# WoojuLee24/OA-DG

Hardware: AMD Instinct MI355X
Metric: images/sec training, Faster R-CNN R50-FPN + OA-DG, 1024x2048 (higher is better)
Workload: dtype bf16

## Files before the change

include/oadg_hip.h:

```cpp
#ifndef OADG_HIP_H
#define OADG_HIP_H

#include <stddef.h>
#include <stdint.h>

#ifdef __cplusplus
extern "C" {
#endif

size_t oadg_supcon_workspace_bytes(int B, int D);
int oadg_supcon_fwd(const float* feats, const int64_t* labels, int B, int D, int n_labels, int ori_size,
                    int rp_size, float temper, int min_samples, float loss_weight, void* workspace,
                    size_t workspace_bytes, float* out_loss, void* stream);
int oadg_supcon_bwd(const int64_t* labels, int B, int D, int n_labels, int ori_size, int rp_size,
                    float temper, float loss_weight, const float* grad_out, void* workspace,
                    size_t workspace_bytes, float* dfeats, void* stream);
int oadg_supcon_status(const void* workspace_host_copy);

size_t oadg_cls_loss_workspace_bytes(void);
int oadg_ce_jsd_fwd(const float* logits, const int64_t* labels, const float* weights, long R, int C,
                    int mode, float avg_factor, float loss_weight, float lambda_jsd, void* workspace,
                    size_t workspace_bytes, float* out3, void* stream);
int oadg_ce_jsd_bwd(const float* logits, const int64_t* labels, const float* weights, long R, int C,
                    int mode, float avg_factor, float loss_weight, float lambda_jsd, const float* grad_out,
// ... 146 lines not shown

int oadg_png_size(const char* path, int* height, int* width);
int oadg_png_decode_bgr(const char* path, uint8_t* out, int H, int W);

int oadg_glass_shuffle_u8(uint8_t* img, int H, int W, int C, int delta, int iters, const int32_t* dxdy);
int oadg_chamfer_l2_5x5(const uint8_t* src, int H, int W, float* dist);

int oadg_resize_bilinear_u8(const uint8_t* src, int H, int W, int C, uint8_t* dst, int Hn, int Wn, void* stream);
int oadg_flip_u8(const uint8_t* src, int H, int W, int C, uint8_t* dst, int direction, void* stream);

int oadg_conv2d_nhwc_bf16(const void* x, const void* w, const float* bias, const void* residual, void* y,
                          const void* zeros16, int N, int H, int W, int C, int K, int R, int S, int stride,
                          int pad, int dil, int relu, void* stream);

int oadg_conv2d_nhwc_bf16_variant(const void* x, const void* w, const float* bias, const void* residual, void* y,
                                  const void* zeros16, int N, int H, int W, int C, int K, int R, int S, int stride,
                                  int pad, int dil, int relu, int variant, void* stream);
int oadg_conv2d_nhwc_bf16_ex(const void* x, const void* w, const float* bias, const void* residual, void* y,
                             const void* zeros16, int N, int H, int W, int C, int K, int R, int S, int stride, int pad,
                             int dil, int relu, int variant, const void* mask, float* colsum_part,
                             const void* mask_bits, void* relu_bits_out, void* stream);
long oadg_conv2d_pixel_tiles(int N, int H, int W, int C, int K, int R, int S, int stride, int pad, int dil,
                             int variant);
int oadg_colsum_reduce(const float* part, long rows, int K, float* out, void* stream);
typedef struct oadg_colsum_job {
    const float* part;
    float* out;
    float* dgamma;
    const float* mean;
    const float* var;
    int rows, K, first_block;
    float eps;
} oadg_colsum_job;
int oadg_colsum_reduce_multi(const oadg_colsum_job* jobs_dev, int n, int total_blocks, void* stream);
int oadg_conv2d_auto_variant(int N, int H, int W, int C, int K, int R, int S, int stride, int pad, int dil);
size_t oadg_conv2d_wgrad_workspace_bytes(int N, int Ho, int Wo, int C, int K, int R, int S);
int oadg_conv2d_wgrad_variant(int N, int Ho, int Wo, int C, int K, int R, int S);
int oadg_conv2d_wgrad_nhwc_bf16(const void* x, const void* dy, float* dw, const void* zeros16, void* workspace,
                                size_t workspace_bytes, int N, int H, int W, int C, int K, int R, int S,
                                int stride, int pad, int dil, void* stream);

int oadg_conv2d_wgrad_parts_nhwc_bf16(const void* x, const void* dy, const void* zeros16, void* workspace,
                                      size_t workspace_bytes, int N, int H, int W, int C, int K, int R, int S,
                                      int stride, int pad, int dil, int* splits, void* stream);
int oadg_prep_conv_weights_bwd_parts(const float* part, int splits, const float* gbias, const float* w,
                                     const float* scale, const float* mean, const float* var, float eps, int K, int C,
// ... 191 lines not shown
```

oa-dg_amd/_lib.py:

```python
import ctypes
import os
from ctypes import (POINTER, Structure, c_char_p, c_double, c_float, c_int, c_int64, c_long, c_size_t, c_void_p)

_HERE = os.path.dirname(os.path.abspath(__file__))
LIB_PATH = os.environ.get('OADG_HIP_LIB') or os.path.join(_HERE, 'csrc', 'liboadg_hip.so')
_lib = None

vp, ci, cf, cl, cs, cd = c_void_p, c_int, c_float, c_long, c_size_t, c_double


class RpnLevel(Structure):
    _fields_ = [('deltas', c_void_p), ('sN', c_long), ('sC', c_long), ('sH', c_long), ('sW', c_long), ('anchors', c_void_p),
                ('scores', c_void_p), ('index', c_void_p), ('H', c_int), ('W', c_int), ('A', c_int), ('k', c_int),
                ('dtype', c_int), ('first', c_int)]


class RpnLossLevel(Structure):
    _fields_ = [('y', c_void_p), ('gy', c_void_p), ('sN', c_long), ('sC', c_long), ('sH', c_long), ('sW', c_long),
                ('H', c_int), ('W', c_int), ('Cy', c_int), ('first', c_long), ('pix0', c_long)]


class RoiAssignImage(Structure):
    _fields_ = [('proposals', c_void_p), ('gt_bboxes', c_void_p), ('gt_labels', c_void_p), ('stride', c_int),
                ('num_gts', c_int)]
# ... 37 lines not shown
                                vp, ci, ci, ci, ci, ci, vp, vp, vp]),
    'oadg_roi_align_bwd': (ci, [POINTER(vp), POINTER(ci), POINTER(ci), POINTER(cf), ci, ci, ci, ci, cf,
                                vp, ci, ci, ci, ci, ci, vp, vp, vp]),
    'oadg_roi_order_keys': (ci, [vp, ci, ci, ci, cf, vp, vp]),
    'oadg_roi_order': (ci, [vp, ci, ci, ci, cf, vp, vp, vp]),
    'oadg_roi_align_bwd_tiles': (ci, [POINTER(vp), POINTER(ci), POINTER(ci), POINTER(cf), ci, ci, ci, cf, vp, ci, ci, ci,
                                      ci, ci, vp, vp, vp, vp, vp]),
    'oadg_rpn_loss_workspace_bytes': (cs, []),
    'oadg_rpn_loss_fwd': (ci, [vp, ci, ci, ci, cl, ci, vp, vp, vp, vp, cf, cf, cf, cf, vp, cs, vp, vp]),
    'oadg_rpn_loss_bwd': (ci, [vp, ci, ci, ci, cl, ci, vp, vp, vp, vp, cf, cf, cf, cf, vp, vp, vp]),
    'oadg_rpn_decode': (ci, [vp, ci, ci, vp, vp, cf, vp, ci, cf, vp, vp, vp, vp]),
    'oadg_rpn_order': (ci, [vp, ci, ci, vp, vp, vp, vp, vp, vp, vp, vp]),
    'oadg_rpn_gather': (ci, [ci, ci, ci, vp, vp, vp, vp, vp, vp, vp]),
    'oadg_rpn_topk_workspace_bytes': (cs, [POINTER(ci), ci, ci, ci]),
    'oadg_rpn_topk': (ci, [POINTER(vp), POINTER(cl), POINTER(ci), ci, ci, ci, ci, POINTER(vp), POINTER(vp), vp, cs, vp]),
    'oadg_nms_workspace_bytes': (cs, [ci, ci]),
    'oadg_nms_batched': (ci, [vp, vp, ci, ci, cf, ci, vp, cs, vp, vp, vp]),
    'oadg_resize_bilinear_u8': (ci, [vp, ci, ci, ci, vp, ci, ci, vp]),
    'oadg_flip_u8': (ci, [vp, ci, ci, ci, vp, ci, vp]),
    'oadg_conv2d_nhwc_bf16': (ci, [vp, vp, vp, vp, vp, vp] + [ci] * 11 + [vp]),
    'oadg_conv2d_auto_variant': (ci, [ci] * 10),
    'oadg_conv2d_nhwc_bf16_ex': (ci, [vp, vp, vp, vp, vp, vp] + [ci] * 12 + [vp, vp, vp, vp, vp]),
    'oadg_conv2d_pixel_tiles': (cl, [ci] * 11),
    'oadg_colsum_reduce': (ci, [vp, cl, ci, vp, vp]),
    'oadg_conv2d_nhwc_bf16_variant': (ci, [vp, vp, vp, vp, vp, vp] + [ci] * 12 + [vp]),
    'oadg_conv2d_wgrad_workspace_bytes': (cs, [ci] * 7),
    'oadg_conv2d_wgrad_variant': (ci, [ci] * 7),
    'oadg_conv2d_wgrad_nhwc_bf16': (ci, [vp, vp, vp, vp, vp, cs] + [ci] * 10 + [vp]),
    'oadg_conv2d_wgrad_parts_nhwc_bf16': (ci, [vp, vp, vp, vp, cs] + [ci] * 10 + [POINTER(ci), vp]),
    'oadg_prep_conv_weights_bwd_parts': (ci, [vp, ci, vp, vp, vp, vp, vp, cf, ci, ci, ci, ci, vp, vp, ci, vp]),
    'oadg_prep_conv_weights': (ci, [vp, vp, vp, vp, vp, cf, vp, ci, ci, ci, ci, vp, vp, vp, vp, ci, ci, vp]),
    'oadg_prep_conv_weights_multi': (ci, [vp, ci, ci, vp]),
    'oadg_prep_conv_weights_multi_blocks': (ci, [ci, ci, ci, ci]),
    'oadg_conv2d_nhwc_bf16_scatter': (ci, [vp, vp, vp, vp, vp, vp] + [ci] * 18 + [vp, vp, vp, vp]),
    'oadg_conv2d_dgrad_s2_nhwc_bf16': (ci, [vp, vp, vp, vp, vp, ci, ci, ci, ci, ci, ci, ci, ci, vp, vp, vp, vp]),
    'oadg_prep_conv_weights_bwd': (ci, [vp, vp, vp, vp, vp, vp, cf, ci, ci, ci, ci, vp, vp, ci, vp]),
    'oadg_relu_bias_bwd_workspace_bytes': (ctypes.c_size_t, [cl, ci]),
    'oadg_relu_bias_bwd': (ci, [vp, ci, vp, vp, vp, vp, ctypes.c_size_t, cl, ci, vp]),
    'oadg_stem_conv7x7s2_nhwc_bf16': (ci, [vp, vp, vp, ci, ci, ci, vp]),
    'oadg_bias_relu_maxpool_nhwc_bf16': (ci, [vp, vp, vp, ci, ci, ci, ci, vp]),
    'oadg_fpn_topdown_fwd': (ci, [vp, vp, vp, ci, ci, ci, ci, ci, ci, vp]),
    'oadg_fpn_topdown_bwd': (ci, [vp, vp, ci, ci, ci, ci, ci, ci, vp]),
    'oadg_max_iou_assign_workspace_bytes': (ctypes.c_size_t, [ci, ci]),
    'oadg_max_iou_assign': (ci, [vp, cl, vp, vp, vp, vp, ci, ci, ci, cf, cf, cf, cf, ci, vp, ctypes.c_size_t, vp, vp, vp,
                                 vp, vp]),
    'oadg_sample_select_workspace_bytes': (ctypes.c_size_t, [ci, cl]),
# ... 101 lines not shown
```

oa-dg_amd/backbones.py:

```python
import torch
import torch.nn as nn
import torch.nn.functional as F
from torch.nn.modules.batchnorm import _BatchNorm

import os

from . import hip_conv
from .layers import Conv2d, build_norm_layer, constant_init, conv_bn, kaiming_init
from .registry import BACKBONES


STEM_KERNEL = os.environ.get('OADG_STEM_KERNEL', '1') == '1'


class Bottleneck(nn.Module):
    expansion = 4

    def __init__(self, inplanes, planes, stride=1, dilation=1, downsample=None, style='pytorch',
                 norm_cfg=dict(type='BN')):
        super().__init__()
        assert style in ('pytorch', 'caffe')
        s1, s2 = (1, stride) if style == 'pytorch' else (stride, 1)
        self.conv1 = Conv2d(inplanes, planes, 1, stride=s1, bias=False)
        _, self.bn1 = build_norm_layer(norm_cfg, planes)
        self.conv2 = Conv2d(planes, planes, 3, stride=s2, padding=dilation, dilation=dilation, bias=False)
        _, self.bn2 = build_norm_layer(norm_cfg, planes)
        self.conv3 = Conv2d(planes, planes * self.expansion, 1, bias=False)
        _, self.bn3 = build_norm_layer(norm_cfg, planes * self.expansion)
        self.relu = nn.ReLU(inplace=True)
        self.downsample = downsample

    def forward(self, x):
        out = hip_conv.frozen_bottleneck(x, self)
        if out is not None:
            return out
        t_in = getattr(x, '_oadg_token', None)
        if hip_conv.tokens_ok(x, self.conv1, self.conv2, self.conv3) and not (self.bn1.training or self.bn2.training
                                                                              or self.bn3.training):
            t_a, t_b, t_out = hip_conv.GradToken(), hip_conv.GradToken(), hip_conv.GradToken()
            if not x.requires_grad or (self.downsample is not None and
                                       not hip_conv.tokens_ok(x, self.downsample[0])):
                t_in = None
            out = conv_bn(x, self.conv1, self.bn1, relu=True, in_token=t_in, out_token=t_a)
            out = conv_bn(out, self.conv2, self.bn2, relu=True, in_token=t_a, out_token=t_b)
            if self.downsample is not None:
                identity = conv_bn(x, self.downsample[0], self.downsample[1], dep_token=t_in)
                out = conv_bn(out, self.conv3, self.bn3, relu=True, residual=identity, in_token=t_b, out_token=t_out)
            else:
                out = conv_bn(out, self.conv3, self.bn3, relu=True, residual=x, in_token=t_b, out_token=t_out,
                              res_token=t_in)
            out._oadg_token = t_out
            return out
        identity = x
        if self.downsample is not None:
            identity = conv_bn(x, self.downsample[0], self.downsample[1])
        out = conv_bn(x, self.conv1, self.bn1, relu=True)
        out = conv_bn(out, self.conv2, self.bn2, relu=True)
        return conv_bn(out, self.conv3, self.bn3, relu=True, residual=identity)


def make_res_layer(inplanes, planes, num_blocks, stride, dilation, style, norm_cfg):
    downsample = None
    if stride != 1 or inplanes != planes * Bottleneck.expansion:
        downsample = nn.Sequential(
            Conv2d(inplanes, planes * Bottleneck.expansion, 1, stride=stride, bias=False),
            build_norm_layer(norm_cfg, planes * Bottleneck.expansion)[1])
    blocks = [Bottleneck(inplanes, planes, stride, dilation, downsample, style, norm_cfg)]
    inplanes = planes * Bottleneck.expansion
    for _ in range(1, num_blocks):
        blocks.append(Bottleneck(inplanes, planes, 1, dilation, None, style, norm_cfg))
    return nn.Sequential(*blocks)


@BACKBONES.register_module()
class ResNet(nn.Module):
    arch_settings = {50: (3, 4, 6, 3), 101: (3, 4, 23, 3), 152: (3, 8, 36, 3)}

    def __init__(self, depth, in_channels=3, stem_channels=None, base_channels=64, num_stages=4,
                 strides=(1, 2, 2, 2), dilations=(1, 1, 1, 1), out_indices=(0, 1, 2, 3), style='pytorch',
                 deep_stem=False, avg_down=False, frozen_stages=-1, conv_cfg=None,
                 norm_cfg=dict(type='BN', requires_grad=True), norm_eval=True, dcn=None,
                 stage_with_dcn=(False, False, False, False), plugins=None, with_cp=False,
                 zero_init_residual=True, pretrained=None, init_cfg=None):
        super().__init__()
        if depth not in self.arch_settings:
            raise KeyError(f'invalid depth {depth} for resnet (bottleneck depths only)')
        assert not deep_stem and not avg_down and dcn is None and plugins is None and not with_cp
        assert 1 <= num_stages <= 4 and len(strides) == len(dilations) == num_stages
        assert max(out_indices) < num_stages
        self.depth, self.out_indices, self.frozen_stages = depth, out_indices, frozen_stages
        self.norm_eval, self.zero_init_residual, self.init_cfg = norm_eval, zero_init_residual, init_cfg
        stem_channels = stem_channels or base_channels
        self.conv1 = Conv2d(in_channels, stem_channels, 7, stride=2, padding=3, bias=False)
        _, self.bn1 = build_norm_layer(norm_cfg, stem_channels)
# ... 101 lines not shown
```

oa-dg_amd/csrc/conv_mfma.hip:

```cpp
#include <algorithm>
#include <vector>
#include "common.h"
#include <type_traits>
#include <stdlib.h>
#include "oadg_hip.h"

namespace {

constexpr int BM = 128, BN = 128, BK = 64;

struct ConvArgs {
    const unsigned short* x;
    const unsigned short* w;
    const float* bias;
    const unsigned short* res;
    unsigned short* y;
    const unsigned short* zeros;
    const unsigned short* mask;
    const unsigned char* bits_in;
    unsigned char* bits_out;
    float* colsum;
    int N, H, W, C, K, R, S, Ho, Wo, stride, pad, dil, relu;
    long M;
    int scatter, OH, OW, osh, osw, oph, opw;
// ... 512 lines not shown
int launch_pw_stream(const ConvArgs& a, hipStream_t st) {
    using Geo = PwGeo<C>;
    const int ncol = a.K / (4 * Geo::KPW);
    const bool res = a.res != nullptr, bin = a.bits_in != nullptr, bout = a.bits_out != nullptr;
#define OADG_PWS(RE, BI, BO)                                                                                       \
    do {                                                                                                           \
        static bool attr = false;                                                                                  \
        if (!attr) {                                                                                               \
            hipError_t e = hipFuncSetAttribute((const void*)conv_pw_stream_kernel<C, RE, BI, BO>,                  \
                                               hipFuncAttributeMaxDynamicSharedMemorySize, Geo::LDS);              \
            if (e != hipSuccess) return (int)e;                                                                    \
            attr = true;                                                                                           \
        }                                                                                                          \
        hipLaunchKernelGGL((conv_pw_stream_kernel<C, RE, BI, BO>), dim3(Geo::GRID), dim3(256), Geo::LDS, st, a, ncol); \
    } while (0)
    if (res && bin && !bout) OADG_PWS(true, true, false);
    else if (res && !bin && bout) OADG_PWS(true, false, true);
    else if (res && !bin && !bout) OADG_PWS(true, false, false);
    else if (!res && bin && !bout) OADG_PWS(false, true, false);
    else if (!res && !bin && bout) OADG_PWS(false, false, true);
    else if (!res && !bin && !bout) OADG_PWS(false, false, false);
    else return OADG_EARG;
#undef OADG_PWS
    return OADG_OK;
}

constexpr int TM = 256, TN = 256;
constexpr int HALF_BYTES = 128 * BK * 2;
constexpr int BUF_BYTES = 4 * HALF_BYTES;

typedef float f32x4v __attribute__((ext_vector_type(4)));

struct TapState {
    int t, r, s, rs, c0;
};

template <bool POST, int NW>
__global__ __launch_bounds__(512) void conv_igemm256_kernel(ConvArgs a) {
    constexpr int TNW = NW * 128;
    extern __shared__ __attribute__((aligned(16))) unsigned char smem[];
    const int tid = threadIdx.x, lane = tid & 63;
    const int wave = __builtin_amdgcn_readfirstlane(tid >> 6);
    const int wr = wave >> 2, wc = wave & 3;
    const int n_tiles = a.K / TNW;
    const long m_tiles = (a.M + TM - 1) / TM;
    const long bid = blockIdx.x;
// ... 363 lines not shown
}
}

extern "C" int oadg_conv2d_nhwc_bf16(const void* x, const void* w, const float* bias, const void* residual,
                                     void* y, const void* zeros16, int N, int H, int W, int C, int K, int R,
                                     int S, int stride, int pad, int dil, int relu, void* stream) {
    return conv_launch(x, w, bias, residual, y, zeros16, N, H, W, C, K, R, S, stride, pad, dil, relu, 0, stream);
}

extern "C" int oadg_conv2d_auto_variant(int N, int H, int W, int C, int K, int R, int S, int stride, int pad, int dil) {
    if (N < 1 || H < 1 || W < 1 || R < 1 || S < 1 || stride < 1 || dil < 1 || pad < 0) return 0;
    if (C % BK != 0 || K % 64 != 0) return 0;
    const int Ho = (H + 2 * pad - dil * (R - 1) - 1) / stride + 1, Wo = (W + 2 * pad - dil * (S - 1) - 1) / stride + 1;
    if (Ho < 1 || Wo < 1) return 0;
    return auto_variant((long)N * Ho * Wo, H, W, C, K, R * S * (C / BK), R, S, stride, pad);
}

extern "C" int oadg_conv2d_nhwc_bf16_ex(const void* x, const void* w, const float* bias, const void* residual,
                                        void* y, const void* zeros16, int N, int H, int W, int C, int K, int R, int S,
                                        int stride, int pad, int dil, int relu, int variant, const void* mask,
                                        float* colsum_part, const void* mask_bits, void* relu_bits_out, void* stream) {
    return conv_launch(x, w, bias, residual, y, zeros16, N, H, W, C, K, R, S, stride, pad, dil, relu, variant, stream,
                       mask, colsum_part, nullptr, mask_bits, relu_bits_out);
}

extern "C" int oadg_conv2d_nhwc_bf16_scatter(const void* x, const void* w, const float* bias, const void* residual,
                                             void* y, const void* zeros16, int N, int H, int W, int C, int K, int R,
                                             int S, int pad, int dil, int relu, int out_h, int out_w, int OH, int OW,
                                             int osh, int osw, int oph, int opw, const void* mask,
                                             float* colsum_part, const void* mask_bits, void* stream) {
    const int sc[8] = {out_h, out_w, OH, OW, osh, osw, oph, opw};
    return conv_launch(x, w, bias, residual, y, zeros16, N, H, W, C, K, R, S, 1, pad, dil, relu, 3, stream, mask,
                       colsum_part, sc, mask_bits, nullptr);
}

extern "C" int oadg_conv2d_dgrad_s2_nhwc_bf16(const void* dy, const void* wt, const void* residual, void* dx,
                                              const void* zeros16, int N, int Ho, int Wo, int K, int C, int R, int H, int W,
                                              const void* mask, float* colsum_part, const void* mask_bits, void* stream) {
    if (!dy || !wt || !dx || !zeros16 || N < 1 || Ho < 1 || Wo < 1 || H < 1 || W < 1 || (R != 3 && R != 1)) return OADG_EARG;
    if (K % BK != 0 || C % 64 != 0 || (mask_bits && C % 8 != 0)) return OADG_EARG;
    static const int cls_tab[4][5] = {{0, 0, 1, 1, 0}, {0, 1, 1, 2, 1}, {1, 0, 2, 1, 3}, {1, 1, 2, 2, 5}};
    S2Args g;
    ConvArgs& a = g.base;
    a.x = (const unsigned short*)dy; a.w = nullptr; a.bias = nullptr; a.res = (const unsigned short*)residual;
    a.y = (unsigned short*)dx; a.zeros = (const unsigned short*)zeros16; a.mask = (const unsigned short*)mask;
    a.bits_in = (const unsigned char*)mask_bits; a.bits_out = nullptr; a.colsum = nullptr;
// ... 1218 lines not shown
```

oa-dg_amd/hip_conv.py:

```python
import ctypes
import os

import numpy as np
import torch

from . import _lib
from ._lib import check, ptr, stream_ptr

_ZEROS = {}
USE_HIP_WGRAD = 'auto'
TIMERS = None
TIMERS_ONLY_VARIANT = None


def _timed(family):
    if TIMERS is None:
        return False
    only = TIMERS_ONLY_VARIANT
    return only is None or family == only or (isinstance(only, (set, frozenset, tuple, list)) and family in only)


def _wgrad_events(x16, gy16, K, R, S):
    if TIMERS is None:
        return None
# ... 831 lines not shown
        cache_on._prepared = (key, out)
    return out


class GradToken:
    __slots__ = ('extra', 'colsum', 'grad_ptr', 'bits', 'armed', 'closed', 'masked')

    def __init__(self, masked=True):
        self.extra = self.colsum = self.grad_ptr = self.bits = None
        self.armed = self.closed = False
        self.masked = masked


RELU_BITS = True
DEPOSIT = True


def y_numel(x, w, stride, pad, dil):
    N, _, H, W = x.shape
    K, _, R, S = w.shape
    return N * K * ((H + 2 * pad - dil * (R - 1) - 1) // stride + 1) * ((W + 2 * pad - dil * (S - 1) - 1) // stride + 1)


class _Conv2dMFMA(torch.autograd.Function):

    @staticmethod
    def forward(ctx, x, wf, bias, residual, wt, stride, pad, dil, relu, in_token, out_token, res_token, dep_token=None,
                res_up=False):
        x16 = _nhwc_bf16(x)
        if in_token is not None and wt is not None and stride == 1:
            in_token.armed = True
        r16 = _nhwc_bf16(residual) if residual is not None else None
        bits = None
        if relu and out_token is not None and RELU_BITS and wf.shape[0] % 8 == 0:
            bits = out_token.bits = torch.empty((y_numel(x16, wf, stride, pad, dil) // 8,), dtype=torch.uint8,
                                                device=x16.device)
        y = conv_forward(x16, wf, bias, r16, stride, pad, dil, relu, bits_out=bits, res_up=bool(res_up))
        ctx.res_up = tuple(r16.shape) if res_up else None
        ctx.save_for_backward(x16, wf, wt, y if relu else None)
        ctx.cfg = (stride, pad, dil, bias is not None, x.dtype, residual.dtype if residual is not None else None)
        ctx.tokens = (in_token, out_token, res_token, dep_token)
        ctx.wtoken = getattr(wf, '_oadg_wtoken', None)
        if ctx.wtoken is not None:
            ctx.wtoken.uses += 1
            ent = ctx.wtoken.entry
            if ent is not None and DEFER_WGRAD and SHARED_GROUP:
                K_, C_, R_, S_ = wf.shape
                work = wgrad_work(y.shape[0], y.shape[2], y.shape[3], C_, K_, R_, S_)
                if ent.expect_step != _STEP:
                    ent.expect_step, ent.expect_jobs, ent.shared = _STEP, 0, []
                if ctx.wtoken.deferrable and 0 < work < WGRAD_SMALL and C_ * R_ * S_ <= 36000 and x16.numel() < 2 ** 32 and \
                        _hip_wgrad(K_, C_, R_, y.shape[0] * y.shape[2] * y.shape[3]):
                    ent.expect_jobs += 1
        return y

    @staticmethod
    def backward(ctx, gy):
        x16, wf, wt, y = ctx.saved_tensors
        stride, pad, dil, has_bias, xdt, rdt = ctx.cfg
        in_token, out_token, res_token, dep_token = ctx.tokens
        K, C, R, S = wf.shape
        want_b = has_bias and ctx.needs_input_grad[2]
        gb = None
        if out_token is not None and out_token.grad_ptr is not None and out_token.grad_ptr == gy.data_ptr() and \
                gy.dtype == torch.bfloat16 and gy.is_contiguous(memory_format=torch.channels_last):
            gb = out_token.colsum if want_b else None
            want_b = False
            if pending_colsum(gb) is not None and not (ctx.wtoken is not None and ctx.wtoken.uses == 1):
                resolve_colsum(gb)
        elif (y is not None or want_b) and gy.dtype in (torch.bfloat16, torch.float32) and K % 8 == 0 and \
                gy.is_contiguous(memory_format=torch.channels_last):
            gy, gb = relu_bias_bwd(gy, y, want_b)
            want_b = False
        else:
            gy = _nhwc_bf16(gy)
            if y is not None:
# ... 29 lines not shown
            need_x = False
        if need_x and wt is not None and stride == 2:
            if in_token is not None and extra is None and in_token.masked:
                mb = in_token.bits
                gx, in_token.colsum = conv_dgrad_s2(gy, wt, x16.shape, R, mask=None if mb is not None else x16,
                                                    want_colsum=True, mask_bits=mb)
                in_token.grad_ptr = gx.data_ptr()
            else:
                gx = conv_dgrad_s2(gy, wt, x16.shape, R)
            need_x = False
        elif need_x and wt is not None:
            if in_token is not None:
                mb = in_token.bits if in_token.masked else None
                gx, in_token.colsum = conv_forward(gy, wt, None, extra, 1, dil * (R - 1) - pad, dil, False,
                                                   mask=x16 if (mb is None and in_token.masked) else None,
                                                   want_colsum=True, mask_bits=mb)
                in_token.grad_ptr = gx.data_ptr()
                extra = None
            else:
                gx = conv_forward(gy, wt, None, None, 1, dil * (R - 1) - pad, dil, False)
            need_x = False
        gw = None
        if need_w and x16.numel() < 2 ** 32 and _hip_wgrad(K, C, R, gy.shape[0] * gy.shape[2] * gy.shape[3]):
            wtok = ctx.wtoken
            work = wgrad_work(gy.shape[0], gy.shape[2], gy.shape[3], C, K, R, S) if DEFER_WGRAD else 0
            if wtok is not None and wtok.uses == 1 and wtok.deferrable and 0 < work < WGRAD_SMALL and C * R * S <= 36000:
                wtok.parts = _WgradJob(x16, gy, K, R, S, stride, pad, dil)
                gw = _dummy_grad(wf)
            elif wtok is not None and wtok.uses == 1 and C * R * S * 4 <= 12000:
                wtok.parts = conv_wgrad_parts(x16, gy, K, R, S, stride, pad, dil)
                gw = _dummy_grad(wf)
            else:
                gw = conv_wgrad(x16, gy, K, R, S, stride, pad, dil)
            need_w = False
            if want_b:
                gb = gy.float().sum((0, 2, 3))
                want_b = False
        if need_x or need_w or want_b:
            outs = torch.ops.aten.convolution_backward(
                gy, x16, wf, [K] if has_bias else None, [stride, stride], [pad, pad], [dil, dil], False, [0, 0],
                1, [need_x, need_w, want_b])
            if gx is None:
                gx = outs[0]
            if outs[1] is not None:
                gw = outs[1]
            if outs[2] is not None:
                gb = outs[2].float()
        if gx is not None and extra is not None:
            gx = gx + extra.to(gx.dtype)
        gres = None
        if rdt is not None and ctx.needs_input_grad[3]:
            if res_token is not None:
                res_token.extra = gy
            else:
                gres = gy.to(rdt)
            if ctx.res_up is not None:
                ts = ctx.res_up
                g16 = _nhwc_bf16(gy)
                gres = torch.empty(ts, dtype=torch.bfloat16, device=gy.device, memory_format=torch.channels_last)
                check(_lib.lib().oadg_fpn_topdown_bwd(ptr(g16), ptr(gres), g16.shape[0], g16.shape[2], g16.shape[3], ts[2],
                                                      ts[3], g16.shape[1], stream_ptr()), 'oadg_fpn_topdown_bwd')
                gres = gres.to(rdt)
        return (gx.to(xdt) if gx is not None else None), gw, gb, gres, None, None, None, None, None, None, None, None, None, None


NARROW_HEAD = os.environ.get('OADG_NARROW_HEAD', '1') == '1'


def narrow_params(w_cat, b_cat):
    KN, C = w_cat.shape[0], w_cat.shape[1]
    with torch.no_grad():
        w16 = torch.zeros((16, C), dtype=torch.bfloat16, device=w_cat.device)
        w16[:KN].copy_(w_cat.detach().reshape(KN, C))
        wt16 = w16.t().contiguous()
        b16 = torch.zeros((16,), dtype=torch.float32, device=w_cat.device)
        if b_cat is not None:
            b16[:KN].copy_(b_cat.detach())
    return w16, wt16, b16


def _n16_launch(kind, M, C, extra_bytes, fn):
    if TIMERS is None or not _timed('n16'):
        return fn()
    e0, e1 = torch.cuda.Event(enable_timing=True), torch.cuda.Event(enable_timing=True)
    e0.record()
    r = fn()
# ... 192 lines not shown
```

Measured before the change: 145.5.

## Fuse consecutive bottleneck 1x1 convs (conv3 + next conv1) into one streaming kernel

```diff
diff --git a/include/oadg_hip.h b/include/oadg_hip.h
--- a/include/oadg_hip.h
+++ b/include/oadg_hip.h
@@ -192,6 +192,11 @@
                              const void* mask_bits, void* relu_bits_out, void* stream);
 long oadg_conv2d_pixel_tiles(int N, int H, int W, int C, int K, int R, int S, int stride, int pad, int dil,
                              int variant);
+int oadg_conv_pw_pair_ok(long M, int C);
+int oadg_conv_pw_pair_nhwc_bf16(const void* x, const void* w1, const float* b1, const void* res, void* t,
+                                const void* t_bits_in, void* t_bits_out, float* t_colsum, const void* w2, const float* b2,
+                                void* y, const void* y_bits_in, void* y_bits_out, float* y_colsum, const void* zeros16,
+                                long M, int C, int bwd, void* stream);
 int oadg_colsum_reduce(const float* part, long rows, int K, float* out, void* stream);
 typedef struct oadg_colsum_job {
     const float* part;
diff --git a/oa-dg_amd/_lib.py b/oa-dg_amd/_lib.py
--- a/oa-dg_amd/_lib.py
+++ b/oa-dg_amd/_lib.py
@@ -83,6 +83,8 @@
     'oadg_conv2d_auto_variant': (ci, [ci] * 10),
     'oadg_conv2d_nhwc_bf16_ex': (ci, [vp, vp, vp, vp, vp, vp] + [ci] * 12 + [vp, vp, vp, vp, vp]),
     'oadg_conv2d_pixel_tiles': (cl, [ci] * 11),
+    'oadg_conv_pw_pair_ok': (ci, [cl, ci]),
+    'oadg_conv_pw_pair_nhwc_bf16': (ci, [vp] * 15 + [cl, ci, ci, vp]),
     'oadg_colsum_reduce': (ci, [vp, cl, ci, vp, vp]),
     'oadg_conv2d_nhwc_bf16_variant': (ci, [vp, vp, vp, vp, vp, vp] + [ci] * 12 + [vp]),
     'oadg_conv2d_wgrad_workspace_bytes': (cs, [ci] * 7),
diff --git a/oa-dg_amd/backbones.py b/oa-dg_amd/backbones.py
--- a/oa-dg_amd/backbones.py
+++ b/oa-dg_amd/backbones.py
@@ -34,29 +34,62 @@
         out = hip_conv.frozen_bottleneck(x, self)
         if out is not None:
             return out
-        t_in = getattr(x, '_oadg_token', None)
-        if hip_conv.tokens_ok(x, self.conv1, self.conv2, self.conv3) and not (self.bn1.training or self.bn2.training
-                                                                              or self.bn3.training):
-            t_a, t_b, t_out = hip_conv.GradToken(), hip_conv.GradToken(), hip_conv.GradToken()
-            if not x.requires_grad or (self.downsample is not None and
-                                       not hip_conv.tokens_ok(x, self.downsample[0])):
-                t_in = None
-            out = conv_bn(x, self.conv1, self.bn1, relu=True, in_token=t_in, out_token=t_a)
-            out = conv_bn(out, self.conv2, self.bn2, relu=True, in_token=t_a, out_token=t_b)
-            if self.downsample is not None:
-                identity = conv_bn(x, self.downsample[0], self.downsample[1], dep_token=t_in)
-                out = conv_bn(out, self.conv3, self.bn3, relu=True, residual=identity, in_token=t_b, out_token=t_out)
-            else:
-                out = conv_bn(out, self.conv3, self.bn3, relu=True, residual=x, in_token=t_b, out_token=t_out,
-                              res_token=t_in)
-            out._oadg_token = t_out
-            return out
+        if self._tokens_path(x):
+            return self.forward_tokens(x)[0]
         identity = x
         if self.downsample is not None:
             identity = conv_bn(x, self.downsample[0], self.downsample[1])
         out = conv_bn(x, self.conv1, self.bn1, relu=True)
         out = conv_bn(out, self.conv2, self.bn2, relu=True)
         return conv_bn(out, self.conv3, self.bn3, relu=True, residual=identity)
+
+    def _tokens_path(self, x):
+        return hip_conv.tokens_ok(x, self.conv1, self.conv2, self.conv3) and not (self.bn1.training or self.bn2.training
+                                                                                   or self.bn3.training)
+
+    def forward_tokens(self, x, carry=None, nxt=None):
+        t_in = getattr(x, '_oadg_token', None)
+        t_b, t_out = hip_conv.GradToken(), hip_conv.GradToken()
+        if not x.requires_grad or (self.downsample is not None and not hip_conv.tokens_ok(x, self.downsample[0])):
+            t_in = None
+        if carry is not None:
+            out, t_a = carry
+        else:
+            t_a = hip_conv.GradToken()
+            out = conv_bn(x, self.conv1, self.bn1, relu=True, in_token=t_in, out_token=t_a)
+        out = conv_bn(out, self.conv2, self.bn2, relu=True, in_token=t_a, out_token=t_b)
+        if self.downsample is not None:
+            identity, res_token = conv_bn(x, self.downsample[0], self.downsample[1], dep_token=t_in), None
+        else:
+            identity, res_token = x, t_in
+        nxt_carry = None
+        if nxt is not None and nxt._tokens_path(out):
+            t_a2 = hip_conv.GradToken()
+            r = hip_conv.pw_pair(out, self, identity, nxt, t_b, t_out, res_token, t_a2)
+            if r is not None:
+                out, h1 = r
+                nxt_carry = (h1, t_a2)
+        if nxt_carry is None:
+            out = conv_bn(out, self.conv3, self.bn3, relu=True, residual=identity, in_token=t_b, out_token=t_out,
+                          res_token=res_token)
+        out._oadg_token = t_out
+        return out, nxt_carry
+
+
+class ResLayer(nn.Sequential):
+
+    def forward(self, x):
+        pairs = hip_conv.pw_pair_plan(self) if (hip_conv.ENABLED and x.is_cuda) else ()
+        if not pairs:
+            return super().forward(x)
+        carry = None
+        for i, blk in enumerate(self):
+            nxt = self[i + 1] if i in pairs else None
+            if carry is None and (nxt is None or not blk._tokens_path(x)):
+                x = blk(x)
+            else:
+                x, carry = blk.forward_tokens(x, carry, nxt)
+        return x
 
 
 def make_res_layer(inplanes, planes, num_blocks, stride, dilation, style, norm_cfg):
@@ -69,7 +102,7 @@
     inplanes = planes * Bottleneck.expansion
     for _ in range(1, num_blocks):
         blocks.append(Bottleneck(inplanes, planes, 1, dilation, None, style, norm_cfg))
-    return nn.Sequential(*blocks)
+    return ResLayer(*blocks)
 
 
 @BACKBONES.register_module()
diff --git a/oa-dg_amd/csrc/conv_mfma.hip b/oa-dg_amd/csrc/conv_mfma.hip
--- a/oa-dg_amd/csrc/conv_mfma.hip
+++ b/oa-dg_amd/csrc/conv_mfma.hip
@@ -558,6 +558,236 @@
     else if (!res && !bin && !bout) OADG_PWS(false, false, false);
     else return OADG_EARG;
 #undef OADG_PWS
+    return OADG_OK;
+}
+
+template <int C>
+struct PwPairGeo {
+    static_assert(C == 128, "pair geometry written for C = 128 (ResNet stage 2)");
+    static constexpr int C4 = 4 * C, SP = 32, NS = 4, NW = 8, RANGES = 256;
+    static constexpr int SUB_BYTES = SP * C * 2, G = SUB_BYTES / (NW * 1024);
+    static constexpr int RT1 = C4 / NW / 16, KS1 = C / 32, CT = SP / 16, KS2 = C4 / 32;
+    static constexpr int NP1 = 4;
+    static constexpr int T_BYTES = SP * C4 * 2, STG2_STRIDE = 16 * 2 + 16, STG2_BYTES = SP * STG2_STRIDE;
+    static constexpr int LDS = NS * SUB_BYTES + 2 * T_BYTES + T_BYTES + NW * STG2_BYTES + (C4 + C) * 4;
+};
+
+template <int C, bool BWD>
+__global__ __launch_bounds__(512, 1) void conv_pw_stream_pair_kernel(ConvArgs a1, ConvArgs a2) {
+    using Geo = PwPairGeo<C>;
+    constexpr int C4 = Geo::C4, SP = Geo::SP, NS = Geo::NS, NW = Geo::NW, SUB_BYTES = Geo::SUB_BYTES, G = Geo::G;
+    constexpr int RT1 = Geo::RT1, KS1 = Geo::KS1, CT = Geo::CT, KS2 = Geo::KS2, NP1 = Geo::NP1;
+    constexpr int T_BYTES = Geo::T_BYTES, STG2_STRIDE = Geo::STG2_STRIDE, STG2_BYTES = Geo::STG2_BYTES;
+    constexpr int R = NP1 + (BWD ? NP1 + 1 : 0), S = NP1 + 1 + (BWD ? 0 : NP1 + 1);
+    static_assert((NS - 2) * G + (NS - 1) * (R + S) <= 63, "vmcnt is a 6-bit counter");
+    extern __shared__ __attribute__((aligned(16))) unsigned char smem[];
+    const int tid = threadIdx.x, lane = tid & 63;
+    const int wave = __builtin_amdgcn_readfirstlane(tid >> 6);
+    const long range = blockIdx.x, ranges = gridDim.x;
+    const long n_sub = a1.M / SP;
+    const int n_it = range < n_sub ? (int)((n_sub - range + ranges - 1) / ranges) : 0;
+    const int kc1 = wave * 64, kc2 = wave * 16;
+    unsigned char* ring = smem;
+    unsigned char* rres = smem + NS * SUB_BYTES + wave * (NP1 * 1024);
+    unsigned char* tt = smem + NS * SUB_BYTES + 2 * T_BYTES;
+    unsigned char* stg2 = tt + T_BYTES + wave * STG2_BYTES;
+    float* sb1 = reinterpret_cast<float*>(tt + T_BYTES + NW * STG2_BYTES) + kc1;
+    float* sb2 = reinterpret_cast<float*>(tt + T_BYTES + NW * STG2_BYTES) + C4 + kc2;
+    float cs1[8] = {0.f, 0.f, 0.f, 0.f, 0.f, 0.f, 0.f, 0.f}, cs2[8] = {0.f, 0.f, 0.f, 0.f, 0.f, 0.f, 0.f, 0.f};
+    const int fr = lane & 15, fq = lane >> 4;
+    const bf16x8 z8 = {0, 0, 0, 0, 0, 0, 0, 0};
+
+    if (n_it > 0) {
+        bf16x8 w1[RT1][KS1], w2[KS2];
+#pragma unroll
+        for (int rt = 0; rt < RT1; ++rt)
+#pragma unroll
+            for (int ks = 0; ks < KS1; ++ks)
+                w1[rt][ks] = *reinterpret_cast<const bf16x8*>(a1.w + (size_t)(kc1 + rt * 16 + fr) * C + ks * 32 + fq * 8);
+#pragma unroll
+        for (int ks = 0; ks < KS2; ++ks)
+            w2[ks] = *reinterpret_cast<const bf16x8*>(a2.w + (size_t)(kc2 + fr) * C4 + ks * 32 + fq * 8);
+        sb1[lane] = a1.bias ? a1.bias[kc1 + lane] : 0.f;
+        if (lane < 16) sb2[lane] = a2.bias ? a2.bias[kc2 + lane] : 0.f;
+
+        int goff[G];
+#pragma unroll
+        for (int g = 0; g < G; ++g) {
+            const int L = (g * NW + wave) * 64 + lane;
+            const int px = L / (C / 8), sl = L % (C / 8);
+            goff[g] = px * C + (sl ^ (px & 15)) * 8;
+        }
+        auto stage = [&](long sub, int slot) {
+#pragma unroll
+            for (int g = 0; g < G; ++g) {
+                const unsigned short* src = sub < n_sub ? a1.x + (size_t)sub * (SP * C) + goff[g] : a1.zeros;
+                glds16(src, ring + slot * SUB_BYTES + (g * NW + wave) * 1024);
+            }
+        };
+        int bbase[CT], bsw[CT], tbase[CT];
+#pragma unroll
+        for (int ct = 0; ct < CT; ++ct) {
+            const int px = ct * 16 + fr;
+            bbase[ct] = px * (C * 2);
+            tbase[ct] = px * (C4 * 2);
+            bsw[ct] = (fq ^ (px & 15)) << 4;
+        }
+        const int ppx = lane >> 3, psl = lane & 7, qpx = lane >> 1, qsl = lane & 1;
+        const size_t lane_off1 = (size_t)ppx * C4 + kc1 + psl * 8, lane_off2 = (size_t)qpx * C + kc2 + qsl * 8;
+        const size_t sub_stride1 = (size_t)SP * C4, row8 = (size_t)8 * C4, sub_stride2 = (size_t)SP * C;
+        unsigned mb1[2][NP1], mb2[2];
+        auto request = [&](long sub, int set) {
+#pragma unroll
+            for (int jj = 0; jj < NP1; ++jj) {
+                const size_t off = (sub < n_sub ? (size_t)sub * sub_stride1 + jj * row8 : 0) + lane_off1;
+                glds16(a1.res + off, rres + set * T_BYTES + jj * 1024);
+                if (BWD) asm volatile("global_load_ubyte %0, %1, off" : "=v"(mb1[set][jj]) : "v"(a1.bits_in + (off >> 3)) : "memory");
+            }
+            if (BWD) {
+                const size_t off = (sub < n_sub ? (size_t)sub * sub_stride2 : 0) + lane_off2;
+                asm volatile("global_load_ubyte %0, %1, off" : "=v"(mb2[set]) : "v"(a2.bits_in + (off >> 3)) : "memory");
+            }
+        };
+
+#pragma unroll
+        for (int p = 0; p < NS - 1; ++p) stage(range + p * ranges, p);
+        request(range, 0);
+
+        auto body = [&](int i, auto set_c) {
+            constexpr int set = decltype(set_c)::value;
+            const long sub = range + i * ranges;
+            OADG_VMCNT((NS - 2) * G + (NS - 1) * (R + S));
+            asm volatile("s_barrier" ::: "memory");
+            stage(sub + (NS - 1) * ranges, (i + NS - 1) % NS);
+            request(sub + ranges, set ^ 1);
+            const unsigned char* at = ring + (i % NS) * SUB_BYTES;
+#pragma unroll
+            for (int ct = 0; ct < CT; ++ct) {
+                f32x4 acc[RT1];
+#pragma unroll
+                for (int rt = 0; rt < RT1; ++rt) acc[rt] = f32x4{0.f, 0.f, 0.f, 0.f};
+#pragma unroll
+                for (int ks = 0; ks < KS1; ++ks) {
+                    const bf16x8 pf = *reinterpret_cast<const bf16x8*>(at + bbase[ct] + (bsw[ct] ^ (ks * 64)));
+#pragma unroll
+                    for (int rt = 0; rt < RT1; ++rt)
+                        acc[rt] = __builtin_amdgcn_mfma_f32_16x16x32_bf16(w1[rt][ks], pf, acc[rt], 0, 0, 0);
+                }
+                const int px = ct * 16 + fr;
+#pragma unroll
+                for (int rt = 0; rt < RT1; ++rt) {
+                    const f32x4 bv = *reinterpret_cast<const f32x4*>(sb1 + rt * 16 + fq * 4);
+                    bf16x4 o;
+#pragma unroll
+                    for (int r = 0; r < 4; ++r) o[r] = (short)f32_to_bf16(acc[rt][r] + bv[r]);
+                    const int sl = (kc1 >> 3) + rt * 2 + (fq >> 1);
+                    *reinterpret_cast<bf16x4*>(tt + px * (C4 * 2) + ((sl ^ (px & 15)) << 4) + (fq & 1) * 8) = o;
+                }
+            }
+            asm volatile("" ::: "memory");
+            OADG_VMCNT(S + G + R);
+            if (BWD) {
+#pragma unroll
+                for (int jj = 0; jj < NP1; ++jj) asm volatile("" : "+v"(mb1[set][jj]));
+                asm volatile("" : "+v"(mb2[set]));
+            }
+#pragma unroll
+            for (int jj = 0; jj < NP1; ++jj) {
+                const int px = ppx + 8 * jj;
+                unsigned char* tp = tt + px * (C4 * 2) + ((((kc1 >> 3) + psl) ^ (px & 15)) << 4);
+                bf16x8 v = *reinterpret_cast<const bf16x8*>(tp);
+                const bf16x8 rv = *reinterpret_cast<const bf16x8*>(rres + set * T_BYTES + jj * 1024 + lane * 16);
+                const size_t off = (size_t)sub * sub_stride1 + jj * row8 + lane_off1;
+                v = finish_piece<true>(a1, v, rv, z8, cs1, BWD ? mb1[set][jj] : 0xffu, off);
+                asm volatile("global_store_dwordx4 %0, %1, off" ::"v"(a1.y + off), "v"(v) : "memory");
+                *reinterpret_cast<bf16x8*>(tp) = v;
+            }
+            asm volatile("s_waitcnt lgkmcnt(0)\n\ts_barrier" ::: "memory");
+            f32x4 acc2[CT];
+#pragma unroll
+            for (int ct = 0; ct < CT; ++ct) acc2[ct] = f32x4{0.f, 0.f, 0.f, 0.f};
+#pragma unroll
+            for (int ks = 0; ks < KS2; ++ks) {
+                bf16x8 pf[CT];
+#pragma unroll
+                for (int ct = 0; ct < CT; ++ct)
+                    pf[ct] = *reinterpret_cast<const bf16x8*>(tt + tbase[ct] + (bsw[ct] ^ (ks * 64)));
+#pragma unroll
+                for (int ct = 0; ct < CT; ++ct)
+                    acc2[ct] = __builtin_amdgcn_mfma_f32_16x16x32_bf16(w2[ks], pf[ct], acc2[ct], 0, 0, 0);
+            }
+            {
+                const f32x4 bv = *reinterpret_cast<const f32x4*>(sb2 + fq * 4);
+#pragma unroll
+                for (int ct = 0; ct < CT; ++ct) {
+                    bf16x4 o;
+#pragma unroll
+                    for (int r = 0; r < 4; ++r) {
+                        float v = acc2[ct][r] + bv[r];
+                        if (a2.relu) v = fmaxf(v, 0.f);
+                        o[r] = (short)f32_to_bf16(v);
+                    }
+                    *reinterpret_cast<bf16x4*>(stg2 + (ct * 16 + fr) * STG2_STRIDE + fq * 8) = o;
+                }
+            }
+            asm volatile("" ::: "memory");
+            {
+                bf16x8 v = *reinterpret_cast<const bf16x8*>(stg2 + qpx * STG2_STRIDE + qsl * 16);
+                const size_t off = (size_t)sub * sub_stride2 + lane_off2;
+                v = finish_piece<BWD>(a2, v, z8, z8, cs2, BWD ? mb2[set] : 0xffu, off);
+                asm volatile("global_store_dwordx4 %0, %1, off" ::"v"(a2.y + off), "v"(v) : "memory");
+            }
+        };
+        OADG_VMCNT(0);
+        for (int i = 0; i < n_it; i += 2) {
+            body(i, std::integral_constant<int, 0>{});
+            if (i + 1 < n_it) body(i + 1, std::integral_constant<int, 1>{});
+        }
+    }
+    if (a1.colsum) {
+#pragma unroll
+        for (int e = 0; e < 8; ++e) {
+            float t = cs1[e];
+#pragma unroll
+            for (int sh = 8; sh < 64; sh <<= 1) t += __shfl_xor(t, sh, 64);
+            cs1[e] = t;
+        }
+        if (lane < 8) {
+#pragma unroll
+            for (int e = 0; e < 8; ++e) a1.colsum[(size_t)range * C4 + kc1 + lane * 8 + e] = cs1[e];
+        }
+    }
+    if (a2.colsum) {
+#pragma unroll
+        for (int e = 0; e < 8; ++e) {
+            float t = cs2[e];
+#pragma unroll
+            for (int sh = 2; sh < 32; sh <<= 1) t += __shfl_xor(t, sh, 64);
+            cs2[e] = t;
+        }
+        if ((lane & 31) < 2) {
+#pragma unroll
+            for (int e = 0; e < 8; ++e) a2.colsum[(size_t)(2 * range + (lane >> 5)) * C + kc2 + (lane & 1) * 8 + e] = cs2[e];
+        }
+    }
+}
+
+bool pw_pair_ok(long M, int C) {
+    return C == 128 && pw_stream_ranges(M, C, 4 * C, 1, 1, 1, 0) == PwPairGeo<128>::RANGES &&
+           pw_stream_ranges(M, 4 * C, C, 1, 1, 1, 0) == 2 * PwPairGeo<128>::RANGES;
+}
+
+template <int C, bool BWD>
+int launch_pw_pair(const ConvArgs& a1, const ConvArgs& a2, hipStream_t st) {
+    using Geo = PwPairGeo<C>;
+    static bool attr = false;
+    if (!attr) {
+        hipError_t e = hipFuncSetAttribute((const void*)conv_pw_stream_pair_kernel<C, BWD>,
+                                           hipFuncAttributeMaxDynamicSharedMemorySize, Geo::LDS);
+        if (e != hipSuccess) return (int)e;
+        attr = true;
+    }
+    hipLaunchKernelGGL((conv_pw_stream_pair_kernel<C, BWD>), dim3(Geo::RANGES), dim3(512), Geo::LDS, st, a1, a2);
     return OADG_OK;
 }
 
@@ -967,6 +1197,33 @@
                                         float* colsum_part, const void* mask_bits, void* relu_bits_out, void* stream) {
     return conv_launch(x, w, bias, residual, y, zeros16, N, H, W, C, K, R, S, stride, pad, dil, relu, variant, stream,
                        mask, colsum_part, nullptr, mask_bits, relu_bits_out);
+}
+
+extern "C" int oadg_conv_pw_pair_ok(long M, int C) { return pw_pair_ok(M, C) ? 1 : 0; }
+
+extern "C" int oadg_conv_pw_pair_nhwc_bf16(const void* x, const void* w1, const float* b1, const void* res, void* t,
+                                           const void* t_bits_in, void* t_bits_out, float* t_colsum, const void* w2,
+                                           const float* b2, void* y, const void* y_bits_in, void* y_bits_out,
+                                           float* y_colsum, const void* zeros16, long M, int C, int bwd, void* stream) {
+    if (!x || !w1 || !res || !t || !w2 || !y || !zeros16 || !pw_pair_ok(M, C)) return OADG_EARG;
+    if (bwd ? (!t_bits_in || !y_bits_in || t_bits_out || y_bits_out)
+            : (!t_bits_out || !y_bits_out || t_bits_in || y_bits_in || t_colsum || y_colsum))
+        return OADG_EARG;
+    ConvArgs a1 = {}, a2 = {};
+    a1.x = (const unsigned short*)x; a1.w = (const unsigned short*)w1; a1.bias = b1; a1.res = (const unsigned short*)res;
+    a1.y = (unsigned short*)t; a1.zeros = (const unsigned short*)zeros16; a1.bits_in = (const unsigned char*)t_bits_in;
+    a1.bits_out = (unsigned char*)t_bits_out; a1.colsum = t_colsum;
+    a1.N = 1; a1.H = 1; a1.W = (int)std::min(M, 0x7fffffffL); a1.C = C; a1.K = 4 * C; a1.R = a1.S = 1; a1.stride = a1.dil = 1;
+    a1.relu = bwd ? 0 : 1; a1.M = M;
+    a2 = a1;
+    a2.x = nullptr; a2.w = (const unsigned short*)w2; a2.bias = b2; a2.res = nullptr; a2.y = (unsigned short*)y;
+    a2.bits_in = (const unsigned char*)y_bits_in; a2.bits_out = (unsigned char*)y_bits_out; a2.colsum = y_colsum;
+    a2.C = 4 * C; a2.K = C;
+    const int rc = bwd ? launch_pw_pair<128, true>(a1, a2, (hipStream_t)stream)
+                       : launch_pw_pair<128, false>(a1, a2, (hipStream_t)stream);
+    if (rc != OADG_OK) return rc;
+    OADG_LAUNCH_CHECK();
+    return OADG_OK;
 }
 
 extern "C" int oadg_conv2d_nhwc_bf16_scatter(const void* x, const void* w, const float* bias, const void* residual,
diff --git a/oa-dg_amd/hip_conv.py b/oa-dg_amd/hip_conv.py
--- a/oa-dg_amd/hip_conv.py
+++ b/oa-dg_amd/hip_conv.py
@@ -877,6 +877,34 @@
     return N * K * ((H + 2 * pad - dil * (R - 1) - 1) // stride + 1) * ((W + 2 * pad - dil * (S - 1) - 1) // stride + 1)
 
 
+def _note_use(wf, x16, y):
+    wtok = getattr(wf, '_oadg_wtoken', None)
+    if wtok is not None:
+        wtok.uses += 1
+        ent = wtok.entry
+        if ent is not None and DEFER_WGRAD and SHARED_GROUP:
+            K_, C_, R_, S_ = wf.shape
+            work = wgrad_work(y.shape[0], y.shape[2], y.shape[3], C_, K_, R_, S_)
+            if ent.expect_step != _STEP:
+                ent.expect_step, ent.expect_jobs, ent.shared = _STEP, 0, []
+            if wtok.deferrable and 0 < work < WGRAD_SMALL and C_ * R_ * S_ <= 36000 and x16.numel() < 2 ** 32 and \
+                    _hip_wgrad(K_, C_, R_, y.shape[0] * y.shape[2] * y.shape[3]):
+                ent.expect_jobs += 1
+    return wtok
+
+
+def _weight_grad(wtok, x16, gy, wf, stride, pad, dil):
+    K, C, R, S = wf.shape
+    work = wgrad_work(gy.shape[0], gy.shape[2], gy.shape[3], C, K, R, S) if DEFER_WGRAD else 0
+    if wtok is not None and wtok.uses == 1 and wtok.deferrable and 0 < work < WGRAD_SMALL and C * R * S <= 36000:
+        wtok.parts = _WgradJob(x16, gy, K, R, S, stride, pad, dil)
+        return _dummy_grad(wf)
+    if wtok is not None and wtok.uses == 1 and C * R * S * 4 <= 12000:
+        wtok.parts = conv_wgrad_parts(x16, gy, K, R, S, stride, pad, dil)
+        return _dummy_grad(wf)
+    return conv_wgrad(x16, gy, K, R, S, stride, pad, dil)
+
+
 class _Conv2dMFMA(torch.autograd.Function):
 
     @staticmethod
@@ -895,18 +923,7 @@
         ctx.save_for_backward(x16, wf, wt, y if relu else None)
         ctx.cfg = (stride, pad, dil, bias is not None, x.dtype, residual.dtype if residual is not None else None)
         ctx.tokens = (in_token, out_token, res_token, dep_token)
-        ctx.wtoken = getattr(wf, '_oadg_wtoken', None)
-        if ctx.wtoken is not None:
-            ctx.wtoken.uses += 1
-            ent = ctx.wtoken.entry
-            if ent is not None and DEFER_WGRAD and SHARED_GROUP:
-                K_, C_, R_, S_ = wf.shape
-                work = wgrad_work(y.shape[0], y.shape[2], y.shape[3], C_, K_, R_, S_)
-                if ent.expect_step != _STEP:
-                    ent.expect_step, ent.expect_jobs, ent.shared = _STEP, 0, []
-                if ctx.wtoken.deferrable and 0 < work < WGRAD_SMALL and C_ * R_ * S_ <= 36000 and x16.numel() < 2 ** 32 and \
-                        _hip_wgrad(K_, C_, R_, y.shape[0] * y.shape[2] * y.shape[3]):
-                    ent.expect_jobs += 1
+        ctx.wtoken = _note_use(wf, x16, y)
         return y
 
     @staticmethod
@@ -982,16 +999,7 @@
             need_x = False
         gw = None
         if need_w and x16.numel() < 2 ** 32 and _hip_wgrad(K, C, R, gy.shape[0] * gy.shape[2] * gy.shape[3]):
-            wtok = ctx.wtoken
-            work = wgrad_work(gy.shape[0], gy.shape[2], gy.shape[3], C, K, R, S) if DEFER_WGRAD else 0
-            if wtok is not None and wtok.uses == 1 and wtok.deferrable and 0 < work < WGRAD_SMALL and C * R * S <= 36000:
-                wtok.parts = _WgradJob(x16, gy, K, R, S, stride, pad, dil)
-                gw = _dummy_grad(wf)
-            elif wtok is not None and wtok.uses == 1 and C * R * S * 4 <= 12000:
-                wtok.parts = conv_wgrad_parts(x16, gy, K, R, S, stride, pad, dil)
-                gw = _dummy_grad(wf)
-            else:
-                gw = conv_wgrad(x16, gy, K, R, S, stride, pad, dil)
+            gw = _weight_grad(ctx.wtoken, x16, gy, wf, stride, pad, dil)
             need_w = False
             if want_b:
                 gb = gy.float().sum((0, 2, 3))
@@ -1022,6 +1030,160 @@
                                                       ts[3], g16.shape[1], stream_ptr()), 'oadg_fpn_topdown_bwd')
                 gres = gres.to(rdt)
         return (gx.to(xdt) if gx is not None else None), gw, gb, gres, None, None, None, None, None, None, None, None, None, None
+
+
+FUSED_PW_PAIR = os.environ.get('OADG_FUSED_PW_PAIR', '1') == '1'
+PW_PAIR_C = (128,)
+
+
+def _plain_1x1(conv):
+    st, pd, dl = _norm3(conv.stride, conv.padding, conv.dilation)
+    return conv.bias is None and st == (1, 1) and pd == (0, 0) and dl == (1, 1) and tuple(conv.weight.shape[2:]) == (1, 1)
+
+
+def _hooked(*mods):
+    return any(m._forward_hooks or m._forward_pre_hooks for m in mods)
+
+
+def pw_pair_candidate(a, b):
+    for blk in (a, b):
+        if not all(hasattr(blk, n) for n in ('conv1', 'conv2', 'conv3', 'bn1', 'bn2', 'bn3', 'downsample')):
+            return False
+    if b.downsample is not None:
+        return False
+    c3, c1 = a.conv3, b.conv1
+    K, C = c3.weight.shape[:2]
+    if C not in PW_PAIR_C or K != 4 * C or tuple(c1.weight.shape[:2]) != (C, K) or not (_plain_1x1(c3) and _plain_1x1(c1)):
+        return False
+    bns = (a.bn1, a.bn2, a.bn3, b.bn1, b.bn2, b.bn3)
+    if any(bn.training for bn in bns) or not (c3.weight.requires_grad and c1.weight.requires_grad):
+        return False
+    mods = [a, b] + [m for blk in (a, b) for m in blk.modules()]
+    return not _hooked(*mods)
+
+
+def pw_pair_plan(blocks):
+    if not FUSED_PW_PAIR:
+        return frozenset()
+    blocks = list(blocks)
+    return frozenset(i for i in range(len(blocks) - 1) if pw_pair_candidate(blocks[i], blocks[i + 1]))
+
+
+class _PwPair(torch.autograd.Function):
+
+    @staticmethod
+    def forward(ctx, h2, w3, b3, identity, w3t, w1, b1, w1t, t_b, t_out, res_token, t_a):
+        L = _lib.lib()
+        x16, r16 = _nhwc_bf16(h2), _nhwc_bf16(identity)
+        N, C, H, W = x16.shape
+        M, C4 = N * H * W, 4 * C
+        t_b.armed = t_out.armed = True
+        out = torch.empty((N, C4, H, W), dtype=torch.bfloat16, device=x16.device, memory_format=torch.channels_last)
+        h1 = torch.empty((N, C, H, W), dtype=torch.bfloat16, device=x16.device, memory_format=torch.channels_last)
+        t_out.bits = torch.empty((M * C4 // 8,), dtype=torch.uint8, device=x16.device)
+        t_a.bits = torch.empty((M * C // 8,), dtype=torch.uint8, device=x16.device)
+        timed = _timed(4)
+        if timed:
+            e0, e1 = torch.cuda.Event(enable_timing=True), torch.cuda.Event(enable_timing=True)
+            e0.record()
+        check(L.oadg_conv_pw_pair_nhwc_bf16(ptr(x16), ptr(w3), ptr(b3), ptr(r16), ptr(out), None, ptr(t_out.bits), None,
+                                            ptr(w1), ptr(b1), ptr(h1), None, ptr(t_a.bits), None, ptr(_zeros(x16.device)),
+                                            M, C, 0, stream_ptr()), 'oadg_conv_pw_pair_nhwc_bf16')
+        if timed:
+            e1.record()
+            _pair_record(e0, e1, N, H, W, C, False)
+        ctx.save_for_backward(x16, w3, w3t, out, w1, w1t, h1)
+        ctx.tokens = (t_b, t_out, res_token, t_a)
+        ctx.rdt, ctx.xdt = identity.dtype, h2.dtype
+        ctx.wtokens = (_note_use(w3, x16, out), _note_use(w1, out, h1))
+        ctx.set_materialize_grads(False)
+        return out, h1
+
+    @staticmethod
+    def backward(ctx, g_out, g_h1):
+        x16, w3, w3t, out, w1, w1t, h1 = ctx.saved_tensors
+        t_b, t_out, res_token, t_a = ctx.tokens
+        wtok3, wtok1 = ctx.wtokens
+        L = _lib.lib()
+        N, C, H, W = x16.shape
+        M, C4 = N * H * W, 4 * C
+        want_b1 = ctx.needs_input_grad[6]
+        gb1 = None
+        if g_h1 is None:
+            g_h1 = torch.zeros_like(h1)
+        if t_a.grad_ptr is not None and t_a.grad_ptr == g_h1.data_ptr() and g_h1.dtype == torch.bfloat16 and \
+                g_h1.is_contiguous(memory_format=torch.channels_last):
+            gb1 = t_a.colsum if want_b1 else None
+            if pending_colsum(gb1) is not None and not (wtok1 is not None and wtok1.uses == 1):
+                resolve_colsum(gb1)
+        elif g_h1.dtype in (torch.bfloat16, torch.float32) and g_h1.is_contiguous(memory_format=torch.channels_last):
+            g_h1, gb1 = relu_bias_bwd(g_h1, h1, want_b1)
+        else:
+            g_h1 = torch.ops.aten.threshold_backward(_nhwc_bf16(g_h1), h1, 0)
+            gb1 = g_h1.float().sum((0, 2, 3)) if want_b1 else None
+        t_a.grad_ptr = t_a.colsum = None
+        extra, t_out.extra = t_out.extra, None
+        t_out.closed = True
+        if g_out is not None:
+            g_out = _nhwc_bf16(g_out)
+            extra = g_out if extra is None else extra + g_out
+        if extra is None:
+            extra = torch.zeros_like(out)
+        extra = _nhwc_bf16(extra)
+        g_i = torch.empty_like(out)
+        g_h2 = torch.empty_like(x16)
+        part_t = torch.empty((256, C4), dtype=torch.float32, device=x16.device)
+        part_y = torch.empty((512, C), dtype=torch.float32, device=x16.device)
+        timed = _timed(4)
+        if timed:
+            e0, e1 = torch.cuda.Event(enable_timing=True), torch.cuda.Event(enable_timing=True)
+            e0.record()
+        check(L.oadg_conv_pw_pair_nhwc_bf16(ptr(g_h1), ptr(w1t), None, ptr(extra), ptr(g_i), ptr(t_out.bits), None,
+                                            ptr(part_t), ptr(w3t), None, ptr(g_h2), ptr(t_b.bits), None, ptr(part_y),
+                                            ptr(_zeros(x16.device)), M, C, 1, stream_ptr()), 'oadg_conv_pw_pair_nhwc_bf16')
+        if timed:
+            e1.record()
+            _pair_record(e0, e1, N, H, W, C, True)
+        gb3 = _colsum(part_t, C4)
+        t_b.colsum = _colsum(part_y, C)
+        t_b.grad_ptr = g_h2.data_ptr()
+        t_out.grad_ptr = t_out.colsum = None
+        if not ctx.needs_input_grad[2]:
+            gb3 = None
+        elif pending_colsum(gb3) is not None and not (wtok3 is not None and wtok3.uses == 1):
+            resolve_colsum(gb3)
+        gw1 = _weight_grad(wtok1, out, g_h1, w1, 1, 0, 1) if ctx.needs_input_grad[5] else None
+        gw3 = _weight_grad(wtok3, x16, g_i, w3, 1, 0, 1) if ctx.needs_input_grad[1] else None
+        gres = None
+        if ctx.needs_input_grad[3]:
+            if res_token is not None:
+                res_token.extra = g_i
+            else:
+                gres = g_i.to(ctx.rdt)
+        return g_h2.to(ctx.xdt), gw3, gb3, gres, None, gw1, gb1, None, None, None, None, None
+
+
+def _pair_record(e0, e1, N, H, W, C, bwd):
+    M, C4 = N * H * W, 4 * C
+    TIMERS.append((e0, e1, 2.0 * 2 * M * C * C4, 2.0 * (M * C + 2 * M * C4 + M * C + 2 * C * C4) + (M * C4 + M * C) / 8.0,
+                   'conv_pw_stream_pair_kernel<%d, %s>' % (C, 'true' if bwd else 'false'),
+                   (N, H, W, C, C4, 1, 1, True, bwd, 1)))
+
+
+def pw_pair(h2, a, identity, b, t_b, t_out, res_token, t_a):
+    if not (ENABLED and FUSED_PW_PAIR and RELU_BITS and h2.is_cuda and h2.dim() == 4 and h2.requires_grad and
+            torch.is_grad_enabled() and (h2.dtype == torch.bfloat16 or torch.is_autocast_enabled())):
+        return None
+    N, C, H, W = h2.shape
+    if tuple(identity.shape) != (N, 4 * C, H, W) or not identity.is_cuda or N * H * W * 4 * C >= 1 << 31 or \
+            not _lib.lib().oadg_conv_pw_pair_ok(N * H * W, C):
+        return None
+    c3, c1 = a.conv3, b.conv1
+    w3, b3, w3t = prepared(c3.weight, a.bn3, None, _wt_useful(h2, 4 * C, C, 1, 0, 1, 1), c3)
+    w1, b1, w1t = prepared(c1.weight, b.bn1, None, _wt_useful(h2, C, 4 * C, 1, 0, 1, 1), c1)
+    if w3t is None or w1t is None or b3 is None or b1 is None:
+        return None
+    return _PwPair.apply(h2, w3, b3, identity, w3t, w1, b1, w1t, t_b, t_out, res_token, t_a)
 
 
 NARROW_HEAD = os.environ.get('OADG_NARROW_HEAD', '1') == '1'
```

Result: no change. 144.8 (median of 6 runs) (-0.5%).
